# retir/Style-Big-GAN

Hardware: AMD Instinct MI355X
Metric: images/sec (G+D step) StyleGAN2-ADA 256x256 bf16 (higher is better)
Workload: dtype bf16; 1 GPU; configs/sg2ada.yaml @ 256x256: sg2_classic G (skip) + D (orig), softplus + R1(0.01)/4, idle Greg slot /16 (G lr x 16/17), global batch 64 = 1 rank(s) x 2 round(s) x batch_gpu 32 (the rounds of a phase evaluated in one pass, minibatch-std groups and loss those of the separate rounds), bf16 from 8x8 up (num_fp16_res 6; the reference recipe defaults to 4), conv_clamp 256, ADA off; global_batch=64, per_rank_batch=64, parallelism=dp1

## Files before the change

### style-big-gan_amd/csrc/conv_k64.hip

```cpp
#include "conv_device.h"
#include <type_traits>

using namespace sbgconv;

namespace {


template <class MF, int BC, int BP, int WGC, int WGP>
__global__ __launch_bounds__(512, 2) void conv_k64_kernel(ConvArgs p, unsigned x_bytes, unsigned w_bytes)
{
    constexpr int NW = 8;
    static_assert(WGC * WGP == NW, "8 waves per workgroup");
    constexpr int WC = BC / WGC, WP = BP / WGP;
    constexpr int TC = WC / 16,  TP = WP / 16;
    static_assert(WC % 32 == 0 && WP % 16 == 0 && BC % 64 == 0 && BP % 64 == 0, "tile shape");
    constexpr int IA = BC / 64;
    constexpr int IB = BP / 64;
    constexpr int NSTAGE = 3;
    constexpr int LEAD = NSTAGE - 1;
    constexpr int A_BYTES = BC * 128, B_BYTES = BP * 128, STAGE = A_BYTES + B_BYTES;

    extern __shared__ __attribute__((aligned(16))) unsigned char smem[];

    const int tid = threadIdx.x, lane = tid & 63;
    const int wave = __builtin_amdgcn_readfirstlane(tid >> 6);
    const bool grpY = wave >= 4;
    const int bid = xcd_tile_order(blockIdx.x, gridDim.x);
    const int c0 = (bid % p.ctiles) * BC, p0 = (bid / p.ctiles) * BP;

    __amdgpu_buffer_rsrc_t xr = __builtin_amdgcn_make_buffer_rsrc((void*)p.x, 0, (int)x_bytes, 0x00020000);
    __amdgpu_buffer_rsrc_t wr = __builtin_amdgcn_make_buffer_rsrc((void*)p.w, 0, (int)w_bytes, 0x00020000);

    const int lrow = dma_lrow(lane);
    const int src_k = dma_src_k(lane, lrow);
    unsigned a_base[IA];
#pragma unroll
    for (int i = 0; i < IA; i++) {
        const int co = c0 + chmap((wave * IA + i) * 8 + lrow);
        a_base[i] = (co < p.Cout) ? (unsigned)(co * (int)p.ws_co + src_k) * 2u : SBG_OOB_OFFSET;
    }
    const int kchunks = (p.Cin + 63) >> 6;
    const int nsteps_all = p.ntaps * kchunks;
    int nsteps = nsteps_all;
    const int tl = lane < p.ntaps ? lane : 0;
    const int tbl_dy = p.tap_dy[tl], tbl_dx = p.tap_dx[tl];
    const int tbl_wtap = p.tap_slab[tl] * (int)p.ws_slab * 2;

    auto issue_w = [&](int t, int chunk, int stage) {
        unsigned char* st = smem + stage * STAGE;
        const int wtap = __builtin_amdgcn_readlane(tbl_wtap, t) + chunk * 128;
        const bool ragged = chunk * 64 + 64 > p.Cin;
#pragma unroll
        for (int i = 0; i < IA; i++) {
            unsigned off = a_base[i];
            if (ragged) off = (chunk * 64 + src_k < p.Cin) ? off : SBG_OOB_OFFSET;
            __builtin_amdgcn_raw_ptr_buffer_load_lds(wr, (lds_void_ptr)(st + (wave * IA + i) * 1024), 16, off, wtap, 0, 0);
        }
    };

    const int wci = wave / WGP, wpi = wave % WGP;
    const int wc = wci * WC, wp = wpi * WP;
    const int fr = lane & 15, fg = lane >> 4;
    const int foff = frag_off(fr, fg);
    float4_t acc[TC][TP];
#pragma unroll
    for (int i = 0; i < TC; i++)
#pragma unroll
        for (int j = 0; j < TP; j++) acc[i][j] = float4_t{0.f, 0.f, 0.f, 0.f};
    short8_t fa[2][TC], fb[2][TP];

    auto read_a = [&](int stage) {
        const unsigned char* sa = smem + stage * STAGE + wc * 128;
#pragma unroll
        for (int ks = 0; ks < 2; ks++)
#pragma unroll
            for (int i = 0; i < TC; i++) fa[ks][i] = *reinterpret_cast<const short8_t*>(sa + i * 16 * 128 + (foff ^ (ks * 64)));
    };
    auto mma = [&]() {
#pragma unroll
        for (int ks = 0; ks < 2; ks++)
#pragma unroll
            for (int i = 0; i < TC; i++)
#pragma unroll
                for (int j = 0; j < TP; j++) acc[i][j] = Mfma<MF>::run(fa[ks][i], fb[ks][j], acc[i][j]);
    };


    {
        int b_iy0[IB], b_ix0[IB]; unsigned b_base[IB];
#pragma unroll
        for (int i = 0; i < IB; i++) {
            const int pix = p0 + (wave * IB + i) * 8 + lrow;
            const bool ok = pix < p.P;
            const int pp = ok ? pix : 0;
            const int ox = pp % p.OW, t = pp / p.OW, oy = t % p.OH, n = t / p.OH;
            b_iy0[i] = ok ? oy * p.stride : -(1 << 28);
            b_ix0[i] = ox * p.stride;
            b_base[i] = (unsigned)(n * (int)p.xs_n + src_k) * 2u;
        }
        unsigned x_off[IB]; int x_tap = -1;
        auto issue_x = [&](int t, int chunk, int stage) {
            unsigned char* st = smem + stage * STAGE + A_BYTES;
            if (t != x_tap) {
                x_tap = t;
                const int dy = __builtin_amdgcn_readlane(tbl_dy, t), dx = __builtin_amdgcn_readlane(tbl_dx, t);
#pragma unroll
                for (int i = 0; i < IB; i++) {
                    const int iy = b_iy0[i] + dy, ix = b_ix0[i] + dx;
                    const bool ok = ((unsigned)iy < (unsigned)p.IH) & ((unsigned)ix < (unsigned)p.IW);
                    x_off[i] = ok ? b_base[i] + (unsigned)(iy * (int)p.xs_h + ix * (int)p.xs_w) * 2u : SBG_OOB_OFFSET;
                }
            }
            const bool ragged = chunk * 64 + 64 > p.Cin;
#pragma unroll
            for (int i = 0; i < IB; i++) {
                unsigned off = x_off[i];
                if (ragged) off = (chunk * 64 + src_k < p.Cin) ? off : SBG_OOB_OFFSET;
                __builtin_amdgcn_raw_ptr_buffer_load_lds(xr, (lds_void_ptr)(st + (wave * IB + i) * 1024), 16, off, chunk * 128, 0, 0);
            }
        };
        auto read_b = [&](int stage) {
            const unsigned char* sb = smem + stage * STAGE + A_BYTES + wp * 128;
#pragma unroll
            for (int ks = 0; ks < 2; ks++)
#pragma unroll
                for (int j = 0; j < TP; j++) fb[ks][j] = *reinterpret_cast<const short8_t*>(sb + j * 16 * 128 + (foff ^ (ks * 64)));
        };
        constexpr int C = IA + IB;
        static_assert(LEAD == 2, "gather pipeline: two steps of loads in flight");
        int s_begin = 0;
        if (p.ksplit > 1) {
            const int per = (nsteps_all + p.ksplit - 1) / p.ksplit;
            s_begin = blockIdx.y * per;
            nsteps = nsteps_all - s_begin < per ? nsteps_all - s_begin : per;
            if (nsteps < 0) nsteps = 0;
        }
        int it = s_begin / kchunks, ic = s_begin - it * kchunks, wstage = 0;
        auto issue_next = [&]() {
            issue_w(it, ic, wstage); issue_x(it, ic, wstage);
            wstage = wstage == NSTAGE - 1 ? 0 : wstage + 1;
            if (++ic == kchunks) { ic = 0; it++; }
        };
        if (nsteps > 0) issue_next();
        if (nsteps > 1) { issue_next(); wait_vmcnt_const<C>(); } else wait_vmcnt_const<0>();
        if (grpY) __builtin_amdgcn_s_barrier();
        int stage = 0;
        for (int s = 0; s < nsteps; s++) {
            if (!grpY) { if (s + 1 < nsteps) wait_vmcnt_const<C>(); else wait_vmcnt_const<0>(); }
            __builtin_amdgcn_s_barrier();
            read_a(stage); read_b(stage);
            if (s + LEAD < nsteps) issue_next();
            if (grpY) { if (s + 2 < nsteps) wait_vmcnt_const<C>(); else wait_vmcnt_const<0>(); }
            __builtin_amdgcn_s_waitcnt(0xC07F);
            __builtin_amdgcn_s_barrier();
            __builtin_amdgcn_sched_barrier(0);
            mma();
            __builtin_amdgcn_sched_barrier(0);
            stage = stage == NSTAGE - 1 ? 0 : stage + 1;
        }
        if (!grpY) __builtin_amdgcn_s_barrier();
    }

    conv_epilogue8<TC, TP>(p, acc, c0 + wc, fg, [&](int j, int& n, int& oy, int& ox) {
        const int pix = p0 + wp + 16 * j + fr;
        const int pp = pix < p.P ? pix : 0;
        ox = pp % p.OW; const int t = pp / p.OW; oy = t % p.OH; n = t / p.OH;
        return pix < p.P;
    });
}

template <class MF, int TH, int TW>
__global__ __launch_bounds__(768, 3) void conv_halo_ld_kernel(ConvArgs p, unsigned x_bytes, unsigned w_bytes)
{
    constexpr int BC = 128, BP = 256, WGP = 4;
    constexpr int WC = 64, WP = 64, TC = 4, TP = 4;
    static_assert(TH * TW == BP, "halo tile = TH x TW pixels");
    constexpr int NSTAGE = 4, STAGE = BC * 128;
    constexpr int PW = TW + 2, PH = TH + 2, NPIX = PW * PH;
    constexpr int HPIECES = (NPIX + 7) / 8, HALO_BYTES = HPIECES * 1024;
    constexpr int NT = 9, SEG = TW / 16;
    constexpr int WPIECES = BC / 8 / 2;
    constexpr int HPL = (HPIECES + 1) / 2;

    extern __shared__ __attribute__((aligned(16))) unsigned char smem[];
    unsigned char* const sH = smem + NSTAGE * STAGE;
    unsigned char* const sP = sH + 2 * HALO_BYTES;
    constexpr int PARAM_BYTES = 3072;

    const int tid = threadIdx.x, lane = tid & 63;
    const int wave = __builtin_amdgcn_readfirstlane(tid >> 6);
    const int bid = xcd_tile_order(blockIdx.x, gridDim.x);
    const int tiles_x = p.OW / TW, tiles_y = p.OH / TH;
    const int ntiles = p.ptiles * p.ctiles, G = gridDim.x;
    const int my_tiles = (ntiles - bid + G - 1) / G;
    const int kchunks = (p.Cin + 63) >> 6;
    const int nslices = my_tiles * kchunks;
    struct TileC { int c0, tn, y0, x0; };
    auto decode = [&](int tile) -> TileC {
        TileC r;
        const int ct_ = tile % p.ctiles; int pt_ = tile / p.ctiles;
        const int tx = pt_ % tiles_x; pt_ /= tiles_x;
        const int ty = pt_ % tiles_y;
        r.c0 = ct_ * BC; r.tn = pt_ / tiles_y; r.y0 = ty * TH; r.x0 = tx * TW;
        return r;
    };
    const TileC gstep = decode(G);
    auto advance = [&](TileC t_) -> TileC {
        t_.c0 += gstep.c0; int carry = t_.c0 >= p.ctiles * BC; t_.c0 -= carry ? p.ctiles * BC : 0;
        t_.x0 += gstep.x0 + (carry ? TW : 0); carry = t_.x0 >= tiles_x * TW; t_.x0 -= carry ? tiles_x * TW : 0;
        t_.y0 += gstep.y0 + (carry ? TH : 0); carry = t_.y0 >= tiles_y * TH; t_.y0 -= carry ? tiles_y * TH : 0;
        t_.tn += gstep.tn + carry;
        return t_;
    };
    const int lrow = dma_lrow(lane);
    const int src_k = dma_src_k(lane, lrow);

    if (wave >= 10) {
        const int lh = wave - 10;
        __amdgpu_buffer_rsrc_t xr = __builtin_amdgcn_make_buffer_rsrc((void*)p.x, 0, (int)x_bytes, 0x00020000);
        auto issue_params = [&](int t_, int buf) {
            const TileC pc = decode(t_);
            unsigned char* dst = sP + buf * PARAM_BYTES;
            if (p.noise) {
                __amdgpu_buffer_rsrc_t nr = __builtin_amdgcn_make_buffer_rsrc((void*)p.noise, 0, 0x7fffffff, 0x00020000);
                constexpr int LPR = TW / 4;
                const int r = lane / LPR, cx = (lane - r * LPR) * 4;
                const unsigned off = (unsigned)(pc.tn * (int)p.noise_sn + (pc.y0 + r) * p.OW + pc.x0 + cx) * 4u;
                __builtin_amdgcn_raw_ptr_buffer_load_lds(nr, (lds_void_ptr)dst, 16, off, 0, 0, 0);
            }
            const int co = pc.c0 + 4 * lane;
            const unsigned okm = 0u - (unsigned)((lane < 32) & (co < p.Cout));
            if (p.bias) {
                __amdgpu_buffer_rsrc_t br_ = __builtin_amdgcn_make_buffer_rsrc((void*)p.bias, 0, 0x7fffffff, 0x00020000);
                __builtin_amdgcn_raw_ptr_buffer_load_lds(br_, (lds_void_ptr)(dst + 1024), 16, (((unsigned)co * 4u) & okm) | (SBG_OOB_OFFSET & ~okm), 0, 0, 0);
            }
            if (p.oscale) {
                __amdgpu_buffer_rsrc_t sr = __builtin_amdgcn_make_buffer_rsrc((void*)p.oscale, 0, 0x7fffffff, 0x00020000);
                __builtin_amdgcn_raw_ptr_buffer_load_lds(sr, (lds_void_ptr)(dst + 2048), 16, (((unsigned)(pc.tn * p.Cout + co) * 4u) & okm) | (SBG_OOB_OFFSET & ~okm), 0, 0, 0);
            }
        };
        int rel[HPL]; unsigned ef[(HPL + 5) / 6];
#pragma unroll
        for (int w_ = 0; w_ < (HPL + 5) / 6; w_++) ef[w_] = 0;
#pragma unroll
        for (int i = 0; i < HPL; i++) {
            const int piece = lh * HPL + i, pp = piece * 8 + lrow;
            const int py = pp / PW, px = pp - py * PW;
            rel[i] = (py * (int)p.xs_h + px * (int)p.xs_w + src_k) * 2;
            const unsigned f = (unsigned)(py == 0) | ((unsigned)(py == PH - 1) << 1) | ((unsigned)(px == 0) << 2) | ((unsigned)(px == PW - 1) << 3)
                             | ((unsigned)((piece >= HPIECES) | (pp >= NPIX)) << 4);
            ef[i / 6] |= f << (5 * (i % 6));
        }
        auto issue_halo = [&](auto i_tag, int hbase, unsigned emask, bool kok, int buf) {
            constexpr int i = decltype(i_tag)::value;
            const int piece = lh * HPL + i;
            if (piece >= HPIECES) return;
            const bool bad = (((ef[i / 6] >> (5 * (i % 6))) & emask) != 0u) | !kok;
            const unsigned off = bad ? SBG_OOB_OFFSET : (unsigned)(rel[i] + hbase);
            __builtin_amdgcn_raw_ptr_buffer_load_lds(xr, (lds_void_ptr)(sH + buf * HALO_BYTES + piece * 1024), 16, off, 0, 0, 0);
        };
        auto halo_base = [&](const TileC& t_, int chunk_) { return (t_.tn * (int)p.xs_n + (t_.y0 - 1) * (int)p.xs_h + (t_.x0 - 1) * (int)p.xs_w + chunk_ * 64) * 2; };
        auto edge_mask = [&](const TileC& t_) {
            const unsigned m = (unsigned)(t_.y0 == 0) | ((unsigned)(t_.y0 + TH == p.IH) << 1) | ((unsigned)(t_.x0 == 0) << 2) | ((unsigned)(t_.x0 + TW == p.IW) << 3) | 16u;
            return (unsigned)__builtin_amdgcn_readfirstlane((int)m);
        };
        int ctile = bid, cchunk = 0, cpar = 0;
        int tile = bid, chunk = 0;
        TileC tc = decode(tile);
        {
            const int hbase = halo_base(tc, 0); const unsigned emask = edge_mask(tc);
            sbg_static_for<HPL>([&](auto it_) { issue_halo(it_, hbase, emask, src_k < p.Cin, 0); });
        }
        constexpr int per = 2;
        for (int c = 0; c < nslices; c++) {
            wait_vmcnt_const<0>();
            __builtin_amdgcn_s_barrier();
            const bool more = c + 1 < nslices;
            if (more) {
                if (++chunk == kchunks) { chunk = 0; tile += G; tc = advance(tc); }
            }
            const int hbase = halo_base(tc, chunk); const unsigned emask = edge_mask(tc);
            const bool kok = chunk * 64 + src_k < p.Cin;
            sbg_static_for<17>([&](auto it_) {
                constexpr int i = decltype(it_)::value;
                if (more) {
                    if constexpr (per * i < HPL)     issue_halo(std::integral_constant<int, (per * i < HPL ? per * i : 0)>{}, hbase, emask, kok, (c + 1) & 1);
                    if constexpr (per * i + 1 < HPL) issue_halo(std::integral_constant<int, (per * i + 1 < HPL ? per * i + 1 : 0)>{}, hbase, emask, kok, (c + 1) & 1);
                }
                if (i == 12 && lh == 0 && p.lds_params && cchunk == kchunks - 1) issue_params(ctile, cpar);
                if (i == 16 && p.lds_params && c + 1 == nslices) wait_vmcnt_const<0>();
                __builtin_amdgcn_s_barrier();
            });
            if (++cchunk == kchunks) { cchunk = 0; ctile += G; cpar ^= 1; }
        }
        __builtin_amdgcn_s_barrier();
        return;
    }
    if (wave >= 8) {
        const int lw = wave - 8;
        __amdgpu_buffer_rsrc_t wr = __builtin_amdgcn_make_buffer_rsrc((void*)p.w, 0, (int)w_bytes, 0x00020000);
        const int tl = lane < p.ntaps ? lane : 0;
        const int tbl_wtap = p.tap_slab[tl] * (int)p.ws_slab * 2;
        unsigned a_base[WPIECES];
        auto weight_rows = [&](int c0_) {
#pragma unroll
            for (int i = 0; i < WPIECES; i++) {
                const int co = c0_ + chmap((lw * WPIECES + i) * 8 + lrow);
                a_base[i] = (co < p.Cout) ? (unsigned)(co * (int)p.ws_co + src_k) * 2u : SBG_OOB_OFFSET;
            }
        };
        int it = 0, ichunk = 0, itile = bid, istage = 0;
        weight_rows(decode(itile).c0);
        unsigned char* st = nullptr; unsigned kokm = 0, wtap = 0;
        auto issue_prep = [&]() {
            st = smem + istage * STAGE + lw * WPIECES * 1024;
            kokm = 0u - (unsigned)(ichunk * 64 + src_k < p.Cin);
            wtap = (unsigned)(__builtin_amdgcn_readlane(tbl_wtap, it) + ichunk * 128);
        };
        const bool whole_k = (p.Cin & 63) == 0;
        auto issue_part = [&](int lo, int hi) {
            if (whole_k) {
#pragma unroll
                for (int i = 0; i < WPIECES; i++)
                    if (i >= lo && i < hi) __builtin_amdgcn_raw_ptr_buffer_load_lds(wr, (lds_void_ptr)(st + i * 1024), 16, a_base[i], wtap, 0, 0);
                return;
            }
#pragma unroll
            for (int i = 0; i < WPIECES; i++) {
                if (i < lo || i >= hi) continue;
                const unsigned okm = kokm & (0u - (unsigned)(a_base[i] != SBG_OOB_OFFSET));
                const unsigned off = ((a_base[i] + wtap) & okm) | (SBG_OOB_OFFSET & ~okm);
                __builtin_amdgcn_raw_ptr_buffer_load_lds(wr, (lds_void_ptr)(st + i * 1024), 16, off, 0, 0, 0);
            }
        };
        auto issue_done = [&]() {
            istage = (istage + 1) & (NSTAGE - 1);
            if (++it == NT) {
                it = 0;
                if (++ichunk == kchunks) { ichunk = 0; itile += G; if (itile < ntiles) weight_rows(decode(itile).c0); }
            }
        };
        auto issue_next = [&]() { issue_prep(); issue_part(0, WPIECES); issue_done(); };
        constexpr bool split = false;
        const int S = nslices * NT;
        int issued = 0;
        for (; issued < 4 && issued < S; issued++) issue_next();
        for (int s = 0; s < S; s++) {
            const int newer = issued - 1 - s;
            if (newer >= 3) wait_vmcnt_const<3 * WPIECES>();
            else if (newer == 2) wait_vmcnt_const<2 * WPIECES>();
            else if (newer == 1) wait_vmcnt_const<1 * WPIECES>();
            else wait_vmcnt_const<0>();
            __builtin_amdgcn_s_barrier();
            const bool go = s >= 1 && issued < S;
            if (go) { issue_prep(); issue_part(0, split ? WPIECES / 2 : WPIECES); }
            __builtin_amdgcn_s_barrier();
            if (go) { if (split) issue_part(WPIECES / 2, WPIECES); issue_done(); issued++; }
            else if (s >= 1 && issued < S) issued++;
        }
        __builtin_amdgcn_s_barrier();
        return;
    }

    const bool grpY = wave >= 4;
    const int wci = wave >> 2, wpi = wave & 3;
    const int wc = wci * WC;
    const int fr = lane & 15, fg = lane >> 4;
    const int foff = frag_off(fr, fg);
    const int tl = lane < p.ntaps ? lane : 0;
    const int tbl_shift = p.tap_dy[tl] * PW + p.tap_dx[tl];
    float4_t acc[TC][TP];
#pragma unroll
    for (int i = 0; i < TC; i++)
#pragma unroll
        for (int j = 0; j < TP; j++) acc[i][j] = float4_t{0.f, 0.f, 0.f, 0.f};
    short8_t fa[2][TC], fb[2][TP];
    int seg_pp[TP];
#pragma unroll
    for (int j = 0; j < TP; j++) {
        const int sg = wpi * TP + j, r = sg / SEG, cseg = (sg - r * SEG) * 16;
        seg_pp[j] = (r + 1) * PW + cseg + fr + 1;
    }
    int stage = 0, par = 0, chunk = 0, tile = bid;
    TileC cur = decode(tile);
    bool pend = false;
    TileC done = cur;
    int tpar = 0, done_par = 0;
    auto epilogue = [&](const TileC& tc) __attribute__((always_inline)) {
        const LdsParams lp{(lds_cfloat*)(sP + done_par * PARAM_BYTES), wc, TW};
        conv_epilogue8<TC, TP, true>(p, acc, tc.c0 + wc, fg, [&](int j, int& n, int& oy, int& ox) {
            const int sg = wpi * TP + j, r = sg / SEG, cseg = (sg - r * SEG) * 16;
            n = tc.tn; oy = tc.y0 + r; ox = tc.x0 + cseg + fr;
            return true;
        }, 0, p.lds_params ? &lp : nullptr, tc.y0, tc.x0);
#pragma unroll
        for (int i = 0; i < TC; i++)
#pragma unroll
            for (int j = 0; j < TP; j++) acc[i][j] = float4_t{0.f, 0.f, 0.f, 0.f};
    };
    if (grpY) __builtin_amdgcn_s_barrier();
    for (int c = 0; c < nslices; c++) {
        const unsigned char* hb = sH + par * HALO_BYTES;
        sbg_static_for<NT>([&](auto tap_tag) {
            constexpr int t = decltype(tap_tag)::value;
            const int shift = __builtin_amdgcn_readlane(tbl_shift, t);
            const unsigned char* sa = smem + stage * STAGE + wc * 128;
            __builtin_amdgcn_s_barrier();
            if (t == 0 && pend) { epilogue(done); pend = false; }
#pragma unroll
            for (int ks = 0; ks < 2; ks++)
#pragma unroll
                for (int i = 0; i < TC; i++) fa[ks][i] = *reinterpret_cast<const short8_t*>(sa + i * 16 * 128 + (foff ^ (ks * 64)));
#pragma unroll
            for (int j = 0; j < TP; j++) {
                const int pp = seg_pp[j] + shift;
                const int o = pp * 128 + ((fg ^ (pp & 7)) << 4);
#pragma unroll
                for (int ks = 0; ks < 2; ks++) fb[ks][j] = *reinterpret_cast<const short8_t*>(hb + (o ^ (ks * 64)));
            }
            __builtin_amdgcn_s_waitcnt(0xC07F);
            __builtin_amdgcn_s_barrier();
            __builtin_amdgcn_sched_barrier(0);
            mma_step<MF>(acc, fa, fb);
            __builtin_amdgcn_sched_barrier(0);
            stage = (stage + 1) & (NSTAGE - 1);
        });
        par ^= 1;
        if (++chunk < kchunks) continue;
        done = cur; done_par = tpar; tpar ^= 1;
        if (grpY && p.lds_params) epilogue(done); else pend = true;
        chunk = 0; tile += G;
        if (tile < ntiles) cur = advance(cur);
    }
    if (pend) epilogue(done);
    if (!grpY) __builtin_amdgcn_s_barrier();
}

template <class MF>
__global__ __launch_bounds__(768, 3) void conv_gather_ld_kernel(ConvArgs p, unsigned x_bytes, unsigned w_bytes)
{
    constexpr int BC = 128, BP = 256, WGP = 4;
    constexpr int WC = 64, WP = 64, TC = 4, TP = 4;
    constexpr int NSTAGE = 3, A_BYTES = BC * 128, B_BYTES = BP * 128, STAGE = A_BYTES + B_BYTES;
    constexpr int WPIECES = BC / 8 / 2;
    constexpr int XPIECES = BP / 8 / 2;

    extern __shared__ __attribute__((aligned(16))) unsigned char smem[];
    const int tid = threadIdx.x, lane = tid & 63;
    const int wave = __builtin_amdgcn_readfirstlane(tid >> 6);
    const int bid = xcd_tile_order(blockIdx.x, gridDim.x);
    const int ntiles = p.ptiles * p.ctiles, G = gridDim.x;
    const int my_tiles = (ntiles - bid + G - 1) / G;
    const int kchunks = (p.Cin + 63) >> 6;
    auto tile_phase = [&](int tile) { const int r = tile / p.ctiles; return (r % p.nphase + (r / p.nphase) / p.ph_rot_div) % p.nphase; };
    int S = 0;
    for (int t_ = bid; t_ < ntiles; t_ += G) S += p.ph_ntaps[tile_phase(t_)] * kchunks;
    const int lrow = dma_lrow(lane);
    const int src_k = dma_src_k(lane, lrow);
    const int tl = lane < p.ntaps ? lane : 0;

    if (wave >= 8) {
        const bool xload = wave >= 10;
        const int lw = (wave - 8) & 1;
        __amdgpu_buffer_rsrc_t xr = __builtin_amdgcn_make_buffer_rsrc((void*)p.x, 0, (int)x_bytes, 0x00020000);
        __amdgpu_buffer_rsrc_t wr = __builtin_amdgcn_make_buffer_rsrc((void*)p.w, 0, (int)w_bytes, 0x00020000);
        const int tbl_dy = p.tap_dy[tl], tbl_dx = p.tap_dx[tl];
        const int tbl_wtap = p.tap_slab[tl] * (int)p.ws_slab * 2;
        unsigned a_base[WPIECES];
        int b_iy0[XPIECES], b_ix0[XPIECES]; unsigned b_base[XPIECES];
        int ph_t0 = 0, ph_nt = 1;
        auto tile_state = [&](int tile) {
            const int ph = tile_phase(tile);
            const int c0 = (tile % p.ctiles) * BC, p0 = (tile / p.ctiles / p.nphase) * BP;
            const int OW_ = p.ph_OW[ph], OH_ = p.ph_OH[ph], P_ = p.ph_P[ph];
            ph_t0 = p.ph_tap0[ph]; ph_nt = p.ph_ntaps[ph];
            if (!xload) {
#pragma unroll
                for (int i = 0; i < WPIECES; i++) {
                    const int co = c0 + chmap((lw * WPIECES + i) * 8 + lrow);
                    a_base[i] = (co < p.Cout) ? (unsigned)(co * (int)p.ws_co + src_k) * 2u : SBG_OOB_OFFSET;
                }
            } else {
#pragma unroll
                for (int i = 0; i < XPIECES; i++) {
                    const int pix = p0 + (lw * XPIECES + i) * 8 + lrow;
                    const bool ok = pix < P_;
                    const int pp = ok ? pix : 0;
                    const int ox = pp % OW_, t = pp / OW_, oy = t % OH_, n = t / OH_;
                    b_iy0[i] = ok ? oy * p.stride : -(1 << 28);
                    b_ix0[i] = ox * p.stride;
                    b_base[i] = (unsigned)(n * (int)p.xs_n + src_k) * 2u;
                }
            }
        };
        int it = 0, ic = 0, itile = bid, istage = 0;
        tile_state(itile);
        auto issue_part = [&](int half) {
            const unsigned kokm = 0u - (unsigned)(ic * 64 + src_k < p.Cin);
            if (!xload) {
                unsigned char* st = smem + istage * STAGE + lw * WPIECES * 1024;
                const unsigned wtap = (unsigned)(__builtin_amdgcn_readlane(tbl_wtap, ph_t0 + it) + ic * 128);
#pragma unroll
                for (int i = 0; i < WPIECES; i++) {
                    if (half >= 0 && (i >= WPIECES / 2) != (half == 1)) continue;
                    const unsigned okm = kokm & (0u - (unsigned)(a_base[i] != SBG_OOB_OFFSET));
                    const unsigned off = ((a_base[i] + wtap) & okm) | (SBG_OOB_OFFSET & ~okm);
                    __builtin_amdgcn_raw_ptr_buffer_load_lds(wr, (lds_void_ptr)(st + i * 1024), 16, off, 0, 0, 0);
                }
            } else {
                unsigned char* st = smem + istage * STAGE + A_BYTES + lw * XPIECES * 1024;
                const int dy = __builtin_amdgcn_readlane(tbl_dy, ph_t0 + it), dx = __builtin_amdgcn_readlane(tbl_dx, ph_t0 + it);
#pragma unroll
                for (int i = 0; i < XPIECES; i++) {
                    if (half >= 0 && (i >= XPIECES / 2) != (half == 1)) continue;
                    const int iy = b_iy0[i] + dy, ix = b_ix0[i] + dx;
                    const unsigned okm = kokm & (0u - (unsigned)(((unsigned)iy < (unsigned)p.IH) & ((unsigned)ix < (unsigned)p.IW)));
                    const unsigned real = b_base[i] + (unsigned)(iy * (int)p.xs_h + ix * (int)p.xs_w + ic * 64) * 2u;
                    const unsigned off = (real & okm) | (SBG_OOB_OFFSET & ~okm);
                    __builtin_amdgcn_raw_ptr_buffer_load_lds(xr, (lds_void_ptr)(st + i * 1024), 16, off, 0, 0, 0);
                }
            }
        };
        auto issue_done = [&]() {
            istage = istage == NSTAGE - 1 ? 0 : istage + 1;
            if (++ic == kchunks) {
                ic = 0;
                if (++it == ph_nt) { it = 0; itile += G; if (itile < ntiles) tile_state(itile); }
            }
        };
        auto issue_next = [&]() { issue_part(-1); issue_done(); };
        constexpr bool split = true;
        int issued = 0;
        for (; issued < NSTAGE && issued < S; issued++) issue_next();
        for (int s = 0; s < S; s++) {
            const int newer = issued - 1 - s;
            if (xload) {
                if (newer >= 2) wait_vmcnt_const<2 * XPIECES>(); else if (newer == 1) wait_vmcnt_const<XPIECES>(); else wait_vmcnt_const<0>();
            } else {
                if (newer >= 2) wait_vmcnt_const<2 * WPIECES>(); else if (newer == 1) wait_vmcnt_const<WPIECES>(); else wait_vmcnt_const<0>();
            }
            __builtin_amdgcn_s_barrier();
            const bool go = s >= 1 && issued < S;
            if (go) issue_part(split ? 0 : -1);
            __builtin_amdgcn_s_barrier();
            if (go) { if (split) issue_part(1); issue_done(); issued++; }
        }
        __builtin_amdgcn_s_barrier();
        return;
    }

    const bool grpY = wave >= 4;
    const int wci = wave >> 2, wpi = wave & 3;
    const int wc = wci * WC, wp = wpi * WP;
    const int fr = lane & 15, fg = lane >> 4;
    const int foff = frag_off(fr, fg);
    float4_t acc[TC][TP];
#pragma unroll
    for (int i = 0; i < TC; i++)
#pragma unroll
        for (int j = 0; j < TP; j++) acc[i][j] = float4_t{0.f, 0.f, 0.f, 0.f};
    short8_t fa[2][TC], fb[2][TP];
    int stage = 0, tile = bid, left = p.ph_ntaps[tile_phase(bid)] * kchunks;
    bool pend = false;
    int done_tile = tile;
    auto epilogue = [&](int t_) __attribute__((always_inline)) {
        const int ph = tile_phase(t_);
        const int c0 = (t_ % p.ctiles) * BC, p0 = (t_ / p.ctiles / p.nphase) * BP;
        const int OW_ = p.ph_OW[ph], OH_ = p.ph_OH[ph], P_ = p.ph_P[ph];
        conv_epilogue8<TC, TP>(p, acc, c0 + wc, fg, [&](int j, int& n, int& oy, int& ox) {
            const int pix = p0 + wp + 16 * j + fr;
            const int pp = pix < P_ ? pix : 0;
            ox = pp % OW_; const int t = pp / OW_; oy = t % OH_; n = t / OH_;
            return pix < P_;
        }, p.ph_yoff[ph]);
#pragma unroll
        for (int i = 0; i < TC; i++)
#pragma unroll
            for (int j = 0; j < TP; j++) acc[i][j] = float4_t{0.f, 0.f, 0.f, 0.f};
    };
    if (grpY) __builtin_amdgcn_s_barrier();
    for (int s = 0; s < S; s++) {
        const unsigned char* sa = smem + stage * STAGE + wc * 128;
        const unsigned char* sb = smem + stage * STAGE + A_BYTES + wp * 128;
        __builtin_amdgcn_s_barrier();
        if (pend) { epilogue(done_tile); pend = false; }
#pragma unroll
        for (int ks = 0; ks < 2; ks++)
#pragma unroll
            for (int i = 0; i < TC; i++) fa[ks][i] = *reinterpret_cast<const short8_t*>(sa + i * 16 * 128 + (foff ^ (ks * 64)));
#pragma unroll
        for (int ks = 0; ks < 2; ks++)
#pragma unroll
            for (int j = 0; j < TP; j++) fb[ks][j] = *reinterpret_cast<const short8_t*>(sb + j * 16 * 128 + (foff ^ (ks * 64)));
        __builtin_amdgcn_s_waitcnt(0xC07F);
        __builtin_amdgcn_s_barrier();
        __builtin_amdgcn_sched_barrier(0);
        mma_step<MF>(acc, fa, fb);
        __builtin_amdgcn_sched_barrier(0);
        stage = stage == NSTAGE - 1 ? 0 : stage + 1;
        if (--left == 0) { pend = true; done_tile = tile; tile += G; if (tile < ntiles) left = p.ph_ntaps[tile_phase(tile)] * kchunks; }
    }
    if (pend) epilogue(done_tile);
    if (!grpY) __builtin_amdgcn_s_barrier();
}

template <class MF>
static int launch_gather_ld(ConvArgs& a, unsigned x_bytes, unsigned w_bytes, hipStream_t stream)
{
    constexpr int lds = 3 * (128 * 128 + 256 * 128);
    a.ctiles = (a.Cout + 127) / 128;
    if (a.nphase <= 1) {
        a.nphase = 1; a.ph_tap0[0] = 0; a.ph_ntaps[0] = a.ntaps; a.ph_OH[0] = a.OH; a.ph_OW[0] = a.OW; a.ph_P[0] = a.P; a.ph_yoff[0] = 0;
    }
    int pmax = 0;
    for (int i = 0; i < a.nphase; i++) if (a.ph_P[i] > pmax) pmax = a.ph_P[i];
    a.ptiles = ((pmax + 255) / 256) * a.nphase;
    int64_t nblk = (int64_t)a.ptiles * a.ctiles;
    if (nblk > INT32_MAX) return sbg_fail(SBG_ERR_INVALID, "conv2d_igemm: grid too large");
    if (nblk > sbg_cu_count()) nblk = sbg_cu_count();
    a.ph_rot_div = (int)(nblk / ((int64_t)a.ctiles * a.nphase)); if (a.ph_rot_div < 1) a.ph_rot_div = 1;
    double macs = 0.0, outpix = 0.0;
    for (int i = 0; i < a.nphase; i++) { macs += (double)a.ph_P[i] * a.ph_ntaps[i]; outpix += a.ph_P[i]; }
    return conv_launch<conv_gather_ld_kernel<MF>>(nblk, 1, 768, lds, stream, 2.0 * macs * a.Cout * (double)a.Cin, conv_prof_bytes(a, outpix),
                                                  {(int)outpix, a.Cout, a.Cin, a.ntaps, a.stride, a.OH, 4128256 + (a.nphase > 1 ? 1000000 * a.nphase : 0)},
                                                  a, x_bytes, w_bytes);
}

template <class MF, int TH, int TW>
static int launch_halo_ld(ConvArgs& a, unsigned x_bytes, unsigned w_bytes, hipStream_t stream)
{
    constexpr int HPIECES = ((TH + 2) * (TW + 2) + 7) / 8;
    constexpr int lds = 4 * 128 * 128 + 2 * HPIECES * 1024 + 2 * 3072;
    {
        const bool plain = conv_is_plain(a);
        const bool fast = ((a.Cout & 7) == 0) && ((((uintptr_t)a.y) & 15) == 0) && (((a.ys_n | a.ys_h | a.ys_w) & 7) == 0)
                          && ((((uintptr_t)a.oscale) & 15) == 0) && ((((uintptr_t)a.bias) & 15) == 0) && a.ydtype != SBG_F16;
        const bool nz_ok = !a.noise || (((((uintptr_t)a.noise) & 15) == 0) && (a.noise_sn & 3) == 0 && (a.OW & 3) == 0
                                        && (int64_t)a.N * (a.noise_sn > 0 ? a.noise_sn : 0) + (int64_t)a.OH * a.OW < (1ll << 28));
        a.lds_params = !plain && fast && nz_ok && (int64_t)a.N * a.Cout < (1ll << 28);
    }
    static_assert(lds <= 160 * 1024, "LDS budget");
    a.ctiles = (a.Cout + 127) / 128;
    a.ptiles = a.N * (a.OH / TH) * (a.OW / TW);
    int64_t nblk = (int64_t)a.ptiles * a.ctiles;
    if (nblk > INT32_MAX) return sbg_fail(SBG_ERR_INVALID, "conv2d_igemm: grid too large");
    if (nblk > sbg_cu_count()) nblk = sbg_cu_count();
    return conv_launch<conv_halo_ld_kernel<MF, TH, TW>>(nblk, 1, 768, lds, stream, 2.0 * a.P * a.Cout * (double)a.Cin * a.ntaps, conv_prof_bytes(a, a.P),
                                                        {a.P, a.Cout, a.Cin, a.ntaps, a.stride, a.OH, 3128256}, a, x_bytes, w_bytes);
}

template <class MF, int BC, int BP, int WGC, int WGP>
static int launch_k64(ConvArgs& a, unsigned x_bytes, unsigned w_bytes, hipStream_t stream)
{
    constexpr int lds = 3 * (BC * 128 + BP * 128);
    static_assert(lds <= 160 * 1024, "LDS budget");
    a.ctiles = (a.Cout + BC - 1) / BC;
    a.ptiles = (a.P + BP - 1) / BP;
    const int64_t nblk = (int64_t)a.ptiles * a.ctiles;
    return conv_launch<conv_k64_kernel<MF, BC, BP, WGC, WGP>>(nblk, (unsigned)(a.ksplit > 1 ? a.ksplit : 1), 512, lds, stream,
                                                              2.0 * a.P * a.Cout * (double)a.Cin * a.ntaps, conv_prof_bytes(a, a.P),
                                                              {a.P, a.Cout, a.Cin, a.ntaps, a.stride, a.OH, 1000000 + BC * 1000 + BP}, a, x_bytes, w_bytes);
}

__global__ __launch_bounds__(256) void conv_ksplit_reduce_kernel(const float* ws, float* y, int64_t n, int ksplit, int accumulate)
{
    const int sub = threadIdx.x & 15;
    const int64_t step = (int64_t)gridDim.x * 16;
    for (int64_t i = (int64_t)blockIdx.x * 16 + (threadIdx.x >> 4); i < n; i += step) {
        float s = 0.f;
        for (int k = sub; k < ksplit; k += 16) s += ws[(int64_t)k * n + i];
        for (int m = 8; m >= 1; m >>= 1) s += __shfl_xor(s, m, 64);
        if (sub == 0) y[i] = accumulate ? y[i] + s : s;
    }
}

__global__ __launch_bounds__(256) void conv_ksplit_reduce_epi_kernel(const float* ws, ConvArgs p, int64_t n, int ksplit)
{
    const int64_t groups = n >> 3;
    const int hw = p.OH * p.OW;
    for (int64_t g = (int64_t)blockIdx.x * 256 + threadIdx.x; g < groups; g += (int64_t)gridDim.x * 256) {
        const int64_t i = g << 3;
        float acc[8] = {0.f, 0.f, 0.f, 0.f, 0.f, 0.f, 0.f, 0.f};
        for (int k = 0; k < ksplit; k++) {
            float v[8];
            Vec8<float>::ld(ws + (int64_t)k * n + i, v);
#pragma unroll
            for (int e = 0; e < 8; e++) acc[e] += v[e];
        }
        const int64_t pix = i / p.Cout; const int co = (int)(i - pix * p.Cout);
        const int img = (int)(pix / hw), pp = (int)(pix - (int64_t)img * hw);
        const float nz = p.noise ? p.noise[(int64_t)img * p.noise_sn + pp] : 0.f;
#pragma unroll
        for (int e = 0; e < 8; e++) acc[e] = tail(p, acc[e], (int64_t)img * p.Cout + co + e, nz + (p.bias ? p.bias[co + e] : 0.f));
        if (p.ydtype == SBG_F32)       Vec8<float>::st((float*)p.y + i, acc);
        else if (p.ydtype == SBG_BF16) Vec8<bf16_s>::st((bf16_s*)p.y + i, acc);
        else                           Vec8<f16_s>::st((f16_s*)p.y + i, acc);
    }
}

template <class MF>
static int dispatch_k64(ConvArgs& a, unsigned xb, unsigned wb, hipStream_t stream)
{
    if (a.nphase > 1) return launch_gather_ld<MF>(a, xb, wb, stream);
    bool halo = a.stride == 1 && a.ntaps == 9 && a.OH == a.IH && a.OW == a.IW;
    for (int t = 0; halo && t < 9; t++) halo = a.tap_dy[t] >= -1 && a.tap_dy[t] <= 1 && a.tap_dx[t] >= -1 && a.tap_dx[t] <= 1;
    const int64_t tiles256 = (int64_t)((a.P + 255) / 256) * ((a.Cout + 127) / 128);
    if (halo && a.Cout > 64 && tiles256 >= 256) {
        if (a.OW % 32 == 0 && a.OH % 8 == 0)  return launch_halo_ld<MF, 8, 32>(a, xb, wb, stream);
        if (a.OW % 16 == 0 && a.OH % 16 == 0) return launch_halo_ld<MF, 16, 16>(a, xb, wb, stream);
    }
    if (a.Cout <= 64) return launch_k64<MF, 64, 256, 1, 8>(a, xb, wb, stream);
    if (a.ksplit > 1) return launch_k64<MF, 128, 128, 2, 4>(a, xb, wb, stream);
    if (tiles256 < 256) return launch_k64<MF, 128, 128, 2, 4>(a, xb, wb, stream);
    const int ksteps = a.ntaps * ((a.Cin + 63) >> 6);
    if (ksteps >= 2 && ksteps <= 8) return launch_gather_ld<MF>(a, xb, wb, stream);
    return launch_k64<MF, 128, 256, 2, 4>(a, xb, wb, stream);
}

}

static int plan_ksplit(const ConvArgs& a, int ksplit)
{
    if (ksplit <= 1 || a.Cout <= 64) return 1;
    const int nsteps = a.ntaps * ((a.Cin + 63) >> 6);
    int k = ksplit;
    if (k > nsteps / 4) k = nsteps / 4;
    return k < 2 ? 1 : k;
}

extern "C" int64_t sbg_conv2d_igemm_workspace(const sbg_conv_params* q)
{
    if (!q || q->ksplit <= 1) return 0;
    return (int64_t)q->ksplit * q->N * q->OH * q->OW * q->Cout * (int64_t)sizeof(float);
}

int sbg_conv_k64_dispatch(ConvArgs& a, bool bf16, int64_t x_bytes, int64_t w_bytes, void* workspace, int ksplit, hipStream_t stream)
{
    if (x_bytes >= (int64_t)SBG_OOB_OFFSET || w_bytes >= (int64_t)SBG_OOB_OFFSET) return -1;
    if (a.xs_n < 0 || a.xs_h < 0 || a.xs_w < 0 || a.ws_slab < 0 || a.ws_co < 0) return -1;
    const unsigned xb = (unsigned)x_bytes, wb = (unsigned)w_bytes;
    const int64_t y_numel = (int64_t)a.P * a.Cout;
    const bool dense_y = a.ys_w == a.Cout && a.ys_h == (int64_t)a.OW * a.Cout && a.ys_n == (int64_t)a.OH * a.OW * a.Cout;
    const bool simple = a.ydtype == SBG_F32 && conv_is_plain(a);
    const bool epi_ok = !a.accumulate && (a.Cout & 7) == 0 && (((uintptr_t)a.y) & 15) == 0;
    const int k = (workspace && dense_y && (simple || epi_ok)) ? plan_ksplit(a, ksplit) : 1;
    if (k > 1) {
        ConvArgs b = a;
        void* y = a.y; const int acc = a.accumulate;
        b.y = workspace; b.accumulate = 0; b.ksplit = k; b.y_split_stride = y_numel;
        b.ydtype = SBG_F32; b.act = SBG_ACT_LINEAR; b.gain = 1.f; b.clamp = -1.f; b.bias = nullptr; b.noise = nullptr; b.oscale = nullptr;
        const int rc = bf16 ? dispatch_k64<bf16_mfma>(b, xb, wb, stream) : dispatch_k64<f16_mfma>(b, xb, wb, stream);
        if (rc != SBG_OK) return rc;
        if (simple) {
            unsigned grid = (unsigned)((y_numel + 15) / 16); if (grid > 4096) grid = 4096;
            SBG_LAUNCH(conv_ksplit_reduce_kernel, dim3(grid), dim3(256), 0, stream, (const float*)workspace, (float*)y, y_numel, k, acc);
        } else {
            unsigned grid = (unsigned)((y_numel / 8 + 255) / 256); if (grid > 4096) grid = 4096; if (grid < 1) grid = 1;
            SBG_LAUNCH(conv_ksplit_reduce_epi_kernel, dim3(grid), dim3(256), 0, stream, (const float*)workspace, a, y_numel, k);
        }
        SBG_HIP_LAUNCH_CHECK();
        return SBG_OK;
    }
    if (bf16) return dispatch_k64<bf16_mfma>(a, xb, wb, stream);
    return dispatch_k64<f16_mfma>(a, xb, wb, stream);
}
```

Before: 623.8 img/s.

## Add two-stage 256x256 k64 conv tile for stride-2 convs with interleaved loads

Adds a two-stage LDS pipeline variant of the k64 implicit-GEMM conv kernel. In it one wave group spreads its next-step global-to-LDS loads across the MFMA groups, and per-pixel offsets are precomputed per tap. Stride-2 convolutions with Cout divisible by 256 and enough tiles to fill the CUs now dispatch to a 256x256 tile that uses it. The larger tile is meant to raise data reuse, and the interleaving is meant to hide load latency with one step of lookahead instead of two. The cost is less latency slack and higher register and LDS pressure, which may hurt occupancy.

```diff
diff --git a/style-big-gan_amd/csrc/conv_k64.hip b/style-big-gan_amd/csrc/conv_k64.hip
--- a/style-big-gan_amd/csrc/conv_k64.hip
+++ b/style-big-gan_amd/csrc/conv_k64.hip
@@ -6,7 +6,7 @@
 namespace {
 
 
-template <class MF, int BC, int BP, int WGC, int WGP>
+template <class MF, int BC, int BP, int WGC, int WGP, int NSTAGE = 3>
 __global__ __launch_bounds__(512, 2) void conv_k64_kernel(ConvArgs p, unsigned x_bytes, unsigned w_bytes)
 {
     constexpr int NW = 8;
@@ -16,8 +16,8 @@
     static_assert(WC % 32 == 0 && WP % 16 == 0 && BC % 64 == 0 && BP % 64 == 0, "tile shape");
     constexpr int IA = BC / 64;
     constexpr int IB = BP / 64;
-    constexpr int NSTAGE = 3;
     constexpr int LEAD = NSTAGE - 1;
+    static_assert(NSTAGE == 2 || NSTAGE == 3, "gather pipeline: one or two steps of loads in flight");
     constexpr int A_BYTES = BC * 128, B_BYTES = BP * 128, STAGE = A_BYTES + B_BYTES;
 
     extern __shared__ __attribute__((aligned(16))) unsigned char smem[];
@@ -127,7 +127,6 @@
                 for (int j = 0; j < TP; j++) fb[ks][j] = *reinterpret_cast<const short8_t*>(sb + j * 16 * 128 + (foff ^ (ks * 64)));
         };
         constexpr int C = IA + IB;
-        static_assert(LEAD == 2, "gather pipeline: two steps of loads in flight");
         int s_begin = 0;
         if (p.ksplit > 1) {
             const int per = (nsteps_all + p.ksplit - 1) / p.ksplit;
@@ -141,6 +140,7 @@
             wstage = wstage == NSTAGE - 1 ? 0 : wstage + 1;
             if (++ic == kchunks) { ic = 0; it++; }
         };
+        if constexpr (LEAD == 2) {
         if (nsteps > 0) issue_next();
         if (nsteps > 1) { issue_next(); wait_vmcnt_const<C>(); } else wait_vmcnt_const<0>();
         if (grpY) __builtin_amdgcn_s_barrier();
@@ -159,6 +159,110 @@
             stage = stage == NSTAGE - 1 ? 0 : stage + 1;
         }
         if (!grpY) __builtin_amdgcn_s_barrier();
+        } else {
+        static_assert(NSTAGE == 2 && LEAD == 1, "two stages");
+        static_assert(IA == 4, "weight pieces of a wave = one 32-row block");
+        const int tbl_dyx = tbl_dy * 65536 | (tbl_dx & 0xffff);
+        unsigned b_org[IB]; int b_yx[IB];
+#pragma unroll
+        for (int i = 0; i < IB; i++) {
+            const int pix = p0 + (wave * IB + i) * 8 + lrow;
+            const bool ok = pix < p.P;
+            const int pp = ok ? pix : 0;
+            const int ox = pp % p.OW, t = pp / p.OW, oy = t % p.OH, n = t / p.OH;
+            b_yx[i] = ((ok ? oy * p.stride : -16384) * 65536) | (ox * p.stride);
+            b_org[i] = (unsigned)(n * (int)p.xs_n + oy * p.stride * (int)p.xs_h + ox * p.stride * (int)p.xs_w + src_k) * 2u;
+        }
+        auto tap_prep = [&](int t) {
+            if (t != x_tap) {
+                x_tap = t;
+                const int dyx = __builtin_amdgcn_readlane(tbl_dyx, t), dy = dyx >> 16, dx = (int)(short)(dyx & 0xffff);
+                const unsigned shift = (unsigned)(dy * (int)p.xs_h + dx * (int)p.xs_w) * 2u;
+#pragma unroll
+                for (int i = 0; i < IB; i++) {
+                    const int iy = (b_yx[i] >> 16) + dy, ix = (b_yx[i] & 0xffff) + dx;
+                    const bool ok = ((unsigned)iy < (unsigned)p.IH) & ((unsigned)ix < (unsigned)p.IW);
+                    x_off[i] = ok ? b_org[i] + shift : SBG_OOB_OFFSET;
+                }
+            }
+        };
+        auto issue_piece = [&](auto k_tag, int t, int chunk, int stg) {
+            constexpr int k = decltype(k_tag)::value;
+            unsigned char* st = smem + stg * STAGE;
+            const bool ragged = chunk * 64 + 64 > p.Cin;
+            if constexpr (k < IA) {
+                const int wtap = __builtin_amdgcn_readlane(tbl_wtap, t) + chunk * 128 + (16 * (k & 1) + 4 * (k >> 1)) * (int)p.ws_co * 2;
+                unsigned off = a_base[0];
+                if (ragged) off = (chunk * 64 + src_k < p.Cin) ? off : SBG_OOB_OFFSET;
+                __builtin_amdgcn_raw_ptr_buffer_load_lds(wr, (lds_void_ptr)(st + (wave * IA + k) * 1024), 16, off, wtap, 0, 0);
+            } else {
+                constexpr int i = k - IA;
+                unsigned off = x_off[i];
+                if (ragged) off = (chunk * 64 + src_k < p.Cin) ? off : SBG_OOB_OFFSET;
+                __builtin_amdgcn_raw_ptr_buffer_load_lds(xr, (lds_void_ptr)(st + A_BYTES + (wave * IB + i) * 1024), 16, off, chunk * 128, 0, 0);
+            }
+        };
+        auto issue_advance = [&]() {
+            wstage ^= 1;
+            if (++ic == kchunks) { ic = 0; it++; }
+        };
+        auto issue_all = [&]() {
+            tap_prep(it);
+            sbg_static_for<C>([&](auto k_tag) { issue_piece(k_tag, it, ic, wstage); });
+            issue_advance();
+        };
+        constexpr int NG = 2 * TC, GPP = NG / C;
+        static_assert(NG % C == 0, "pieces spread evenly over the MFMA groups");
+        auto mma_issue = [&]() {
+            tap_prep(it);
+            sbg_static_for<NG>([&](auto q_tag) {
+                constexpr int q = decltype(q_tag)::value, ks = q / TC, i = q % TC;
+#pragma unroll
+                for (int j = 0; j < TP; j++) acc[i][j] = Mfma<MF>::run(fa[ks][i], fb[ks][j], acc[i][j]);
+                if constexpr ((q + 1) % GPP == 0) {
+                    __builtin_amdgcn_sched_barrier(0);
+                    issue_piece(std::integral_constant<int, (q + 1) / GPP - 1>{}, it, ic, wstage);
+                    __builtin_amdgcn_sched_barrier(0);
+                }
+            });
+            issue_advance();
+        };
+        if (nsteps > 0) issue_all();
+        int stage = 0;
+        if (!grpY) {
+            for (int s = 0; s < nsteps; s++) {
+                wait_vmcnt_const<0>();
+                __builtin_amdgcn_s_barrier();
+                read_a(stage); read_b(stage);
+                if (s + 1 < nsteps) issue_all();
+                __builtin_amdgcn_s_waitcnt(0xC07F);
+                __builtin_amdgcn_s_barrier();
+                __builtin_amdgcn_sched_barrier(0);
+                mma();
+                __builtin_amdgcn_sched_barrier(0);
+                stage ^= 1;
+            }
+            __builtin_amdgcn_s_barrier();
+        } else {
+            if (nsteps > 1) { issue_all(); wait_vmcnt_const<C>(); } else wait_vmcnt_const<0>();
+            __builtin_amdgcn_s_barrier();
+            auto y_step = [&](auto more_tag) {
+                constexpr bool more = decltype(more_tag)::value;
+                __builtin_amdgcn_s_barrier();
+                read_a(stage); read_b(stage);
+                wait_vmcnt_const<0>();
+                __builtin_amdgcn_s_waitcnt(0xC07F);
+                __builtin_amdgcn_s_barrier();
+                __builtin_amdgcn_sched_barrier(0);
+                if constexpr (more) mma_issue(); else mma();
+                __builtin_amdgcn_sched_barrier(0);
+                stage ^= 1;
+            };
+            int s = 0;
+            for (; s + 2 < nsteps; s++) y_step(std::true_type{});
+            for (; s < nsteps; s++) y_step(std::false_type{});
+        }
+        }
     }
 
     conv_epilogue8<TC, TP>(p, acc, c0 + wc, fg, [&](int j, int& n, int& oy, int& ox) {
@@ -649,15 +753,15 @@
                                                         {a.P, a.Cout, a.Cin, a.ntaps, a.stride, a.OH, 3128256}, a, x_bytes, w_bytes);
 }
 
-template <class MF, int BC, int BP, int WGC, int WGP>
+template <class MF, int BC, int BP, int WGC, int WGP, int NSTAGE = 3>
 static int launch_k64(ConvArgs& a, unsigned x_bytes, unsigned w_bytes, hipStream_t stream)
 {
-    constexpr int lds = 3 * (BC * 128 + BP * 128);
+    constexpr int lds = NSTAGE * (BC * 128 + BP * 128);
     static_assert(lds <= 160 * 1024, "LDS budget");
     a.ctiles = (a.Cout + BC - 1) / BC;
     a.ptiles = (a.P + BP - 1) / BP;
     const int64_t nblk = (int64_t)a.ptiles * a.ctiles;
-    return conv_launch<conv_k64_kernel<MF, BC, BP, WGC, WGP>>(nblk, (unsigned)(a.ksplit > 1 ? a.ksplit : 1), 512, lds, stream,
+    return conv_launch<conv_k64_kernel<MF, BC, BP, WGC, WGP, NSTAGE>>(nblk, (unsigned)(a.ksplit > 1 ? a.ksplit : 1), 512, lds, stream,
                                                               2.0 * a.P * a.Cout * (double)a.Cin * a.ntaps, conv_prof_bytes(a, a.P),
                                                               {a.P, a.Cout, a.Cin, a.ntaps, a.stride, a.OH, 1000000 + BC * 1000 + BP}, a, x_bytes, w_bytes);
 }
@@ -714,6 +818,8 @@
     if (tiles256 < 256) return launch_k64<MF, 128, 128, 2, 4>(a, xb, wb, stream);
     const int ksteps = a.ntaps * ((a.Cin + 63) >> 6);
     if (ksteps >= 2 && ksteps <= 8) return launch_gather_ld<MF>(a, xb, wb, stream);
+    if (a.stride == 2 && a.Cout % 256 == 0 && (a.OH - 1) * 2 + 8 < 32768 && (a.OW - 1) * 2 + 8 < 32768 && (int64_t)((a.P + 255) / 256) * (a.Cout / 256) >= sbg_cu_count())
+        return launch_k64<MF, 256, 256, 2, 4, 2>(a, xb, wb, stream);
     return launch_k64<MF, 128, 256, 2, 4>(a, xb, wb, stream);
 }
 
```

New measurement: 630.6 img/s (median of 6 runs). +1.1%, better.
